# qingxu-thu/INSR-PDE

Hardware: AMD Instinct MI355X
Metric: collocation-points/sec/timestep (incl. ∇/Δ residual + Adam) at 1/2/4/8 GPUs (higher is better)
Workload: dtype fp32

## Files before the change

### include/insr_siren.h

```cpp
#ifndef INSR_SIREN_H
#define INSR_SIREN_H

#ifdef __cplusplus
extern "C" {
#endif

#define INSR_MODE_VALUE 0
#define INSR_MODE_GRAD  1
#define INSR_MODE_LAP   2
#define INSR_MODE_MASK  0xF
#define INSR_MODE_PREC_SHIFT 4
#define INSR_JET_PREC(p) (((p) + 1) << INSR_MODE_PREC_SHIFT)
#define INSR_MODE_BPREC_SHIFT 12
#define INSR_JET_BPREC(p) (((p) + 1) << INSR_MODE_BPREC_SHIFT)
#define INSR_MODE_WSPLIT (1 << 8)
#define INSR_MODE_WIDE128 (1 << 9)
#define INSR_MODE_POLICY_SHIFT 16
#define INSR_JET_POLICY(p) (((p) + 1) << INSR_MODE_POLICY_SHIFT)
#define INSR_MODE_F16_SHIFT 19
#define INSR_JET_BWD_F16(m) (((m) + 1) << INSR_MODE_F16_SHIFT)
#define INSR_MODE_TILES_SHIFT 23
#define INSR_TILES_CODE(t) ((t) == 4 ? 3 : ((t) == 2 ? 2 : ((t) == 1 ? 1 : 0)))
#define INSR_MINB_256 0
#define INSR_MINB_512 1
#define INSR_MINB_128 2
#define INSR_MINB_1024 3
#define INSR_JET_TILES(f, b, minb) \
  ((INSR_TILES_CODE(f) | (INSR_TILES_CODE(b) << 2) | ((minb) << 4)) << INSR_MODE_TILES_SHIFT)

#define INSR_EINVAL   (-1)
#define INSR_EWIDTH   (-2)
#define INSR_ENOCOMM  (-3)
#define INSR_ECAPTURE (-4)
#define INSR_ERANGE   (-5)
#define INSR_ECOMM_BASE 1000

int insr_version(void);

const char* insr_build_id(void);

long insr_siren_param_count(int d_in, int d_out, int num_hidden, int width);

long insr_siren_wsplit_offset(int d_in, int d_out, int num_hidden, int width);
long insr_siren_wsplit_floats(int num_hidden, int width);
int insr_siren_wsplit(float* params, int d_in, int d_out, int num_hidden, int width, void* stream);
int insr_siren_wsplit_status(const float* params, int d_in, int d_out, int num_hidden, int width, void* stream);

int insr_siren_supported(int d_in, int d_out, int num_hidden, int width, int mode);

long insr_jet_act_bytes(long n_points, int d_in, int num_hidden, int width, int mode);

long insr_jet_partial_bytes(long n_points, int d_in, int d_out, int num_hidden, int width, int mode);

int insr_siren_jet_fwd(const float* x, long n_points, int d_in, int d_out, int num_hidden,
                       int width, int mode, const float* params, float* y, float* dy, float* lap,
                       float* act, void* stream);

#define INSR_MAX_FWD_JOBS 6
typedef struct InsrJetJob {
  const float* x;
  const float* params;
  float* y;
  float* dy;
  float* lap;
  float* act;
  long n;
  int d_out;
} InsrJetJob;
#define INSR_MIX_ADVECT 3
int insr_siren_jet_fwd_mixed(const InsrJetJob* jobs, const int* modes, const float* scalars, int n_jobs, int d_in,
                             int d_out, int num_hidden, int width, int prec_mode, void* stream);
int insr_siren_jet_fwd_multi(const InsrJetJob* jobs, int n_jobs, int d_in, int d_out,
                             int num_hidden, int width, int mode, void* stream);

int insr_siren_jet_bwd(const float* x, long n_points, int d_in, int d_out, int num_hidden,
                       int width, int mode, const float* params, const float* act,
                       const float* gy, const float* gdy, const float* glap, float* partial,
                       void* stream);

// ... 228 lines not shown
```

### insr-pde_amd/base/_native.py

```python
import contextlib
import ctypes
import os
import threading

import torch

_HERE = os.path.dirname(os.path.abspath(__file__))
LIB_PATH = os.environ.get("INSR_HIP_LIB", os.path.join(os.path.dirname(_HERE), "lib", "libinsr_hip.so"))

MODE_VALUE, MODE_GRAD, MODE_LAP = 0, 1, 2
MODE_MASK, MODE_PREC_SHIFT = 0xF, 4
MODE_WSPLIT = 1 << 8
PREC_F32, PREC_BF16X6, PREC_BF16X3, PREC_BF16, PREC_F16X3 = 0, 1, 2, 3, 4
PRECISIONS = {"fp32": PREC_F32, "bf16x6": PREC_BF16X6, "bf16x3": PREC_BF16X3, "bf16": PREC_BF16,
              "f16x3": PREC_F16X3}


def jet_prec(p):
    return (int(p) + 1) << MODE_PREC_SHIFT


MODE_BPREC_SHIFT = 12


# ... 94 lines not shown
    "insr_siren_jet_fwd": (_I, [_P, _L, _I, _I, _I, _I, _I, _P, _P, _P, _P, _P, _P]),
    "insr_siren_jet_fwd_multi": (_I, [_P, _I, _I, _I, _I, _I, _I, _P]),
    "insr_siren_jet_bwd": (_I, [_P, _L, _I, _I, _I, _I, _I, _P, _P, _P, _P, _P, _P, _P]),
    "insr_jet_partial_blocks": (_I, [_L, _I, _I, _I]),
    "insr_siren_jet_bwd_grad": (_I, [_P, _L, _I, _I, _I, _I, _I, _P, _P, _P, _P, _P, _P, _P, _I, _P]),
    "insr_jet_bwd_work_bytes": (_L, [_L, _I, _I, _I, _I, _I]),
    "insr_siren_jet_bwd_grad_multi": (_I, [_P, _I, _I, _I, _I, _I, _I, _P, _P, _P, _I, _P]),
    "insr_jet_bwd_multi_work_bytes": (_L, [_P, _I, _I, _I, _I, _I, _I]),
    "insr_siren_jet_bwd_multi_rows": (_I, [_P, _I, _I, _I, _I, _I, _I, _P, _P, _P]),
    "insr_siren_jet_bwd_multi_sweep": (_I, [_P, _I, _I, _I, _I, _I, _I, _P, _P, _P]),
    "insr_jet_bwd_is_wide": (_I, [_L, _I, _I, _I]),
    "insr_jet_bwd_path": (_I, [_L, _I, _I, _I, _I, _I]),
    "insr_jet_bwd_kernel": (_I, [_L, _I, _I, _I, _I, _I]),
    "insr_comm_available": (_I, []),
    "insr_comm_id_bytes": (_L, []),
    "insr_comm_unique_id": (_I, [_P]),
    "insr_comm_init": (_I, [_P, _I, _I, _P]),
    "insr_comm_allreduce_sum": (_I, [_P, _P, _L, _P]),
    "insr_comm_destroy": (_I, [_P]),
    "insr_jet_split_tiles": (_I, [_L, _I, _I, _I, _I]),
    "insr_sq_loss_work_floats": (_L, []),
    "insr_svd_energy_work_floats": (_L, []),
    "insr_svd_energy_fwd": (_I, [_P, _L, _I, _F, _F, _P, _P, _P]),
    "insr_svd_energy_bwd": (_I, [_P, _L, _I, _F, _F, _P, _P, _P]),
    "insr_elastic_work_floats": (_L, []),
    "insr_elastic_energy": (_I, [_P, _P, _P]),
    "insr_sq_loss_fwd": (_I, [_I, _P, _P, _P, _P, _L, _I, _F, _F, _F, _F, _F, _P, _P, _P]),
    "insr_sq_loss_group": (_I, [_P, _I, _P, _P]),
    "insr_axpy_clamp": (_I, [_P, _P, _F, _F, _F, _P, _L, _P]),
    "insr_siren_wsplit_offset": (_L, [_I, _I, _I, _I]),
    "insr_siren_wsplit_floats": (_L, [_I, _I]),
    "insr_siren_wsplit": (_I, [_P, _I, _I, _I, _I, _P]),
    "insr_siren_wsplit_status": (_I, [_P, _I, _I, _I, _I, _P]),
    "insr_siren_jet_fwd_mixed": (_I, [_P, _P, _P, _I, _I, _I, _I, _I, _I, _P]),
    "insr_adam_step_nets": (_I, [_I, _P, _P, _P, _P, _P, _P, _P, _F, _F, _F, _I, _P]),
    "insr_adam_plateau_step_nets": (_I, [_I, _P, _P, _P, _P, _P, _P, _P, _F, _F, _F, _P, _I, _P]),
    "insr_adam_step_partials": (_I, [_P, _I, _L, _P, _I, _P, _P, _P, _L, _P, _P, _F, _F, _F, _P, _I, _P]),
    "insr_siren_jet_bwd_grad_adam": (_I, [_P, _L, _I, _I, _I, _I, _I, _P, _P, _P, _P, _P, _P, _P, _I, _I, _P, _P, _P,
                                          _F, _F, _F, _P, _I, _P]),
    "insr_jet_wide_launch_threads": (_I, [_L, _I, _I, _I, _I, _I, _P]),
    "insr_sq_loss_bwd": (_I, [_I, _P, _P, _P, _P, _L, _I, _F, _F, _F, _F, _F, _P, _P, _P, _P, _P, _P]),
    "insr_reduce_partials": (_I, [_P, _I, _L, _P, _I, _P]),
    "insr_reduce_partials_strided": (_I, [_P, _I, _L, _L, _P, _I, _P]),
    "insr_jet_partial_stride": (_L, [_I, _I, _I, _I]),
    "insr_adam_prepare": (_I, [_P, _F, _F, _P]),
    "insr_plateau_step": (_I, [_P, _P, _I, _I, _P]),
    "insr_adam_step_multi": (_I, [_I, _P, _P, _P, _P, _P, _P, _F, _F, _F, _I, _P]),
    "insr_sampler_state_bytes": (_L, []),
    "insr_sample_boxes": (_I, [_P, _I, _I, ctypes.c_ulonglong, _P, _P]),
    "insr_sample_boxes_rep": (_I, [_P, _I, _I, _I, _P, ctypes.c_ulonglong, _P, _P]),
    "insr_advect1d_rows": (_L, [_L]),
    "insr_advect1d_iteration": (_I, [_P, _P, _I, _I, _L, _L, _P, _P, _F, _F, _F, _F, ctypes.c_ulonglong, _P, _P,
                                     _P, _L, _P, _P, _P]),
    "insr_adam_step": (_I, [_P, _P, _P, _P, _L, _P, _F, _F, _F, _P]),
    "insr_jet_bwd_seed_rows": (_I, [_L, _I, _I, _I, _I, _I]),
    "insr_siren_jet_bwd_seeded": (_I, [_P, _L, _I, _I, _I, _I, _I, _P, _P, _P, _P, _P, _P, _I, _P, _P, _P]),
    "insr_reduce_partials_fin": (_I, [_P, _I, _L, _L, _P, _I, _P, _P]),
    "insr_adam_step_partials_fin": (_I, [_P, _I, _L, _P, _I, _P, _P, _P, _L, _P, _P, _F, _F, _F, _P, _I, _P, _P]),
    "insr_siren_jet_bwd_grad_adam_fin": (_I, [_P, _L, _I, _I, _I, _I, _I, _P, _P, _P, _I, _P, _P, _P, _F, _F, _F, _P,
                                              _I, _P, _P]),
}


MAX_FWD_JOBS = 6


# ... 127 lines not shown
```

### insr-pde_amd/csrc/capi.hip

```cpp
#include <cstdlib>
#include <map>
#include <mutex>
#include <tuple>

#include "jet_common.hpp"
#include "optim.hpp"

namespace insr {

int streams_for(int din, int mode) {
  if (mode == INSR_MODE_VALUE) return 1;
  if (mode == INSR_MODE_GRAD) return 1 + din;
  if (mode == INSR_MODE_LAP) return 2 + din;
  return -1;
}

int nt_for(int width) {
  if (width == 32) return 2;
  if (width == 64) return 4;
  if (width == 128) return 8;
  if (width == 256) return 16;
  return -1;
}

// ... 463 lines not shown
  bool resident(long n, int L) const { return use_resident(n, S, NT, lap, nqb, L, k); }
  bool recompute(int L) const { return use_fb(S, NT, lap, nqb, L, k); }
  bool resident_f16(long n, int L) const { return resident(n, L) && use_resident_f16(n, S, NT, lap, nqb, L, k); }
  int path(long n, int L) const { return recompute(L) ? 3 : (resident(n, L) ? 2 : (wide(n) ? 1 : 0)); }
};

}

using namespace insr;

extern "C" {

int insr_version(void) { return 300; }

long insr_siren_param_count(int din, int dout, int L, int W) {
  return (long)W * din + W + (long)L * ((long)W * W + W) + (long)dout * W + dout;
}

long insr_jet_partial_stride(int din, int dout, int L, int W) {
  return (insr_siren_param_count(din, dout, L, W) + 3) & ~3L;
}

long insr_siren_wsplit_offset(int din, int dout, int L, int W) {
  if (!shape_ok(din, dout, L, W, 0)) return INSR_EINVAL;
  return wsplit_offset(din, dout, L, W);
}
long insr_siren_wsplit_floats(int L, int W) {
  if (L < 0 || nt_for(W) < 0) return INSR_EINVAL;
  return wsplit_total_floats(L, W);
}
int insr_siren_wsplit(float* params, int din, int dout, int L, int W, void* stream) {
  if (!params || !shape_ok(din, dout, L, W, 0)) return INSR_EINVAL;
  return wsplit_launch(params, din, dout, L, W, params + wsplit_offset(din, dout, L, W), (hipStream_t)stream);
}

namespace {
struct Scratch {
  void* ptr = nullptr;
  size_t bytes = 0;
};
std::mutex g_scratch_mu;
std::map<std::tuple<int, hipStream_t, int>, Scratch> g_scratch;
}

static const float* with_planes(const float* params, int din, int dout, int L, int W, int mode, hipStream_t st,
                                int slot, int* rc) {
  *rc = 0;
  if ((mode & INSR_MODE_WSPLIT) || L < 1) return params;
  const long pc = insr_siren_param_count(din, dout, L, W);
  const size_t bytes = (size_t)(wsplit_offset(din, dout, L, W) + wsplit_total_floats(L, W)) * sizeof(float);
  int dev = 0;
  (void)hipGetDevice(&dev);
  std::lock_guard<std::mutex> lk(g_scratch_mu);
  Scratch& e = g_scratch[std::make_tuple(dev, st, slot)];
  if (e.bytes < bytes) {
    hipStreamCaptureStatus cs = hipStreamCaptureStatusNone;
    (void)hipStreamIsCapturing(st, &cs);
    if (cs != hipStreamCaptureStatusNone) {
      *rc = INSR_ECAPTURE;
      return nullptr;
    }
    if (e.ptr) (void)hipFree(e.ptr);
    e.ptr = nullptr;
    e.bytes = 0;
    if (hipMalloc(&e.ptr, bytes) != hipSuccess) {
      *rc = (int)hipErrorOutOfMemory;
// ... 892 lines not shown
```

### insr-pde_amd/csrc/jet_common.hpp

```cpp
#pragma once
#include <hip/hip_runtime.h>
#include <stdint.h>

#include "../../include/insr_siren.h"

typedef float floatx4 __attribute__((ext_vector_type(4)));

#define OMEGA 30.0f
#define OMEGA2 900.0f
#define OMEGA3 27000.0f

namespace insr {


__host__ __device__ inline long act_tiles(long n) { return ((n + 63) / 64) * 4; }

__device__ __forceinline__ floatx4 mfma4(float a, float b, floatx4 c) {
  return __builtin_amdgcn_mfma_f32_16x16x4f32(a, b, c, 0, 0, 0);
}

__host__ __device__ inline long hidden_off(int din, int W, int j) {
  return (long)W * din + W + (long)(j - 1) * ((long)W * W + W);
}
__host__ __device__ inline long out_off(int din, int W, int L) {
// ... 19 lines not shown
__host__ __device__ inline long wsplit_total_floats(int L, int W) { return 5L * L * W * W + 4; }

inline int device_cus() {
  static const int c = [] {
    int dev = 0, v = 0;
    (void)hipGetDevice(&dev);
    return (hipDeviceGetAttribute(&v, hipDeviceAttributeMultiprocessorCount, dev) != hipSuccess || v <= 0) ? 256 : v;
  }();
  return c;
}

__device__ __forceinline__ float* act_base(float* act, int layer, int ntiles, int tile, int S, int NT) {
  return act + ((long)layer * ntiles + tile) * (long)(S * NT) * 256;
}
__device__ __forceinline__ const float* act_base(const float* act, int layer, int ntiles, int tile, int S,
                                                 int NT) {
  return act + ((long)layer * ntiles + tile) * (long)(S * NT) * 256;
}

template <int CTRL>
__device__ __forceinline__ float add_dpp(float v) {
  const int o = __builtin_amdgcn_update_dpp(0, __builtin_bit_cast(int, v), CTRL, 0xF, 0xF, false);
  return v + __builtin_bit_cast(float, o);
}

__device__ __forceinline__ float sum16(float v) {
  v = add_dpp<0xB1>(v);
  v = add_dpp<0x4E>(v);
  v = add_dpp<0x141>(v);
  v = add_dpp<0x140>(v);
  return v;
}

constexpr float kFastArgMax = 8192.0f;

__device__ __forceinline__ float revs_reduced(float x) {
  const float n = rintf(x * 0.15915494309189535f);
  float r = fmaf(-n, 6.28125f, x);
  r = fmaf(-n, 1.9353071795864769e-3f, r);
  return r * 0.15915494309189535f;
}

__device__ __forceinline__ void sincos_fast(float x, float& s, float& c) {
  const float t = revs_reduced(x);
  s = __builtin_amdgcn_sinf(t);
  c = __builtin_amdgcn_cosf(t);
}

__device__ __forceinline__ float sin_fast(float x) { return __builtin_amdgcn_sinf(revs_reduced(x)); }

__device__ __forceinline__ bool wave_any_big(float amax) {
  return __any(amax > kFastArgMax);
}

template <int CTRL>
__device__ __forceinline__ float max_dpp(float v) {
  const int o = __builtin_amdgcn_update_dpp(0, __builtin_bit_cast(int, v), CTRL, 0xF, 0xF, false);
  return fmaxf(v, __builtin_bit_cast(float, o));
}
__device__ __forceinline__ float wave_max_nn(float v) {
  v = max_dpp<0xB1>(v);
  v = max_dpp<0x4E>(v);
  v = max_dpp<0x141>(v);
  v = max_dpp<0x140>(v);
  const int b = __builtin_bit_cast(int, v);
  const unsigned r0 = (unsigned)__builtin_amdgcn_readlane(b, 0), r1 = (unsigned)__builtin_amdgcn_readlane(b, 16);
  const unsigned r2 = (unsigned)__builtin_amdgcn_readlane(b, 32), r3 = (unsigned)__builtin_amdgcn_readlane(b, 48);
  const unsigned m01 = r0 > r1 ? r0 : r1, m23 = r2 > r3 ? r2 : r3;
  return __builtin_bit_cast(float, m01 > m23 ? m01 : m23);
}

__device__ __forceinline__ float wave_max(float v) {
#pragma unroll
  for (int o = 32; o >= 1; o >>= 1) v = fmaxf(v, __shfl_xor(v, o, 64));
  return v;
}


template <int NT, int S, bool LAP, bool FAST>
__device__ __forceinline__ void sine_jet_impl(floatx4 (&a)[NT][S]) {
  constexpr int NTAN = LAP ? S - 2 : S - 1;
#pragma unroll
  for (int rt = 0; rt < NT; ++rt) {
#pragma unroll
    for (int r = 0; r < 4; ++r) {
      const float arg = OMEGA * a[rt][0][r];
      float sn, cs;
      if constexpr (S == 1) {
        if constexpr (FAST) sn = sin_fast(arg); else sn = sinf(arg);
        a[rt][0][r] = sn;
        continue;
      }
      if constexpr (FAST) sincos_fast(arg, sn, cs); else sincosf(arg, &sn, &cs);
      const float wc = OMEGA * cs;
      if constexpr (LAP) {
        float t2 = 0.f;
#pragma unroll
        for (int i = 0; i < NTAN; ++i) t2 = fmaf(a[rt][1 + i][r], a[rt][1 + i][r], t2);
        a[rt][S - 1][r] = wc * a[rt][S - 1][r] - OMEGA2 * sn * t2;
      }
#pragma unroll
      for (int i = 0; i < NTAN; ++i) a[rt][1 + i][r] *= wc;
// ... 336 lines not shown
  const float* gdy[kBwdJobs];
  const float* glap[kBwdJobs];
  int n[kBwdJobs];
  int nbal[kBwdJobs];
  int first[kBwdJobs + 1];
  int njobs;
  SeedTab seeds;
};
template <int NQ>
int dispatch_bwd_q(int NT, int S, bool LAP, int T, const BwdJobsX6* jobs, int din, int dout, int L,
                   const float* prm, float* part, long P, hipStream_t st);
struct AdamArgs {
  float* p = nullptr;
  float* m = nullptr;
  float* v = nullptr;
  float* st = nullptr;
  const float* loss = nullptr;
  int patience = 0;
  float b1 = 0.f, b2 = 0.f, eps = 0.f;
  int shape[4] = {0, 0, 0, 0};
  LossFin fin;
};

struct FbJobs;
template <int NQ>
int dispatch_wide_bwd_q(int NT, int S, bool LAP, const FbJobs& J, int N, int din, int dout, int L, const float* prm,
                        float* work, float* grad, int accumulate, int f16, int phases, const AdamArgs& A,
                        hipStream_t st);
long wide_work_floats(long n, int din, int dout, int L, int W, int S);
template <int NQ>
int dispatch_fwd_mixed_q(int NT, int din, const InsrJetJob* jobs, const int* modes, const float* scalars, int njobs,
                         int dout, int L, hipStream_t st);
int wsplit_launch(const float* prm, int din, int dout, int L, int W, float* planes, hipStream_t st);
void wide_launch_threads(long n, int din, int dout, int L, int W, int S, long* out);
int dispatch_resident_bwd(int S, bool LAP, int L, const float* x, int N, int din, int dout, const float* prm,
                          const float* act, const float* gy, const float* gdy, const float* glap, float* work,
                          float* grad, int accumulate, hipStream_t st);
long resident_work_floats(long n, int din, int dout, int L);
int resident_blocks(long n);

struct FbJobs {
  const float* x[kBwdJobs];
  const float* act[kBwdJobs];
  const float* gy[kBwdJobs];
  const float* gdy[kBwdJobs];
  const float* glap[kBwdJobs];
  int n[kBwdJobs];
  int tstart[kBwdJobs + 1];
  int njobs;
  SeedTab seeds;
};
constexpr int kFbSeedTiles = 24;
int dispatch_fb_bwd(int S, bool LAP, int L, const FbJobs& J, int din, int dout, const float* prm, float* work,
                    float* grad, int accumulate, int saved, int phases, const AdamArgs& A, hipStream_t st);
bool fb_supported(int S, bool LAP, int L);
bool fb_saved_supported(int S, bool LAP, int L);
long fb_work_floats(long tiles, int din, int dout, int L);
int fb_launch_blocks(long tiles);

#define INSR_DISPATCH(NTV, FN, ...)                \
  switch (S * 2 + (LAP ? 1 : 0)) {                 \
    case 2: return FN<NTV, 1, false>(__VA_ARGS__); \
    case 4: return FN<NTV, 2, false>(__VA_ARGS__); \
    case 6: return FN<NTV, 3, false>(__VA_ARGS__); \
    case 8: return FN<NTV, 4, false>(__VA_ARGS__); \
    case 7: return FN<NTV, 3, true>(__VA_ARGS__);  \
// ... 7 lines not shown
```

### insr-pde_amd/csrc/jet_fb.hpp

```cpp
#pragma once
#include <type_traits>

#include "jet_x6w.hpp"

namespace insr {

constexpr int kFbSmallMax = 1412;

#ifdef INSR_STAMPS
constexpr int kFbStampPts = 32;
static __device__ unsigned long long g_fb_stamps[8 * 8 * kFbStampPts];
#define FB_STAMP(k)                                                                                     \
  do {                                                                                                 \
    if (blockIdx.x == 0 && lane == 0 && tile - t0 < 8)                                                 \
      g_fb_stamps[((wave * 8 + (tile - t0)) * kFbStampPts) + (k)] = __builtin_amdgcn_s_memtime();     \
  } while (0)
#else
#define FB_STAMP(k) \
  do {              \
  } while (0)
#endif

template <int S, int L, int ZR, bool SAVED = false, bool SEED = false>
struct FbGeo {
  using BG = X6BwdGeo<4, 8>;
  static constexpr int NZL = (!SAVED && (L - ZR) > 0) ? (L - ZR) : 0;
  static constexpr size_t P_BYTES = (size_t)S * BG::ZSET * 2;
  static constexpr size_t H_BYTES = (size_t)S * BG::ZSET * 2;
  static constexpr size_t ZS_BYTES = (size_t)NZL * S * 8 * 64 * 16;
  static constexpr int SW_FLOATS = 128 * 3 + 128 + L * 128 + 3 * 128;
  static constexpr size_t SW_OFF = P_BYTES + H_BYTES + ZS_BYTES;
  static constexpr size_t SACC_OFF = SW_OFF + (size_t)SW_FLOATS * 4;
  static constexpr size_t SEED_OFF = SACC_OFF + (size_t)kFbSmallMax * 4;
  static constexpr size_t MX_OFF = SEED_OFF + (size_t)S * 3 * 16 * 4;
  static constexpr size_t SSEED_OFF = MX_OFF + 2 * 5 * 8 * 4;
  static constexpr size_t BYTES = SSEED_OFF + (SEED ? ((size_t)kFbSeedTiles * S * 48 + 8 * INSR_SEED_MAX) * 4 : 0);
};

struct FbSinCos {
  floatx4 s, c;
};
__device__ __noinline__ FbSinCos fb_sincos_libm(floatx4 z) {
  FbSinCos o;
#pragma unroll
  for (int r = 0; r < 4; ++r) {
    float a, b;
    sincosf(OMEGA * z[r], &a, &b);
    o.s[r] = a;
    o.c[r] = b;
  }
  return o;
}
__device__ __forceinline__ void fb_sincos(const floatx4& z, floatx4& s, floatx4& c) {
  float amax = 0.f;
#pragma unroll
  for (int r = 0; r < 4; ++r) amax = fmaxf(amax, fabsf(OMEGA * z[r]));
  if (wave_any_big(amax)) {
    const FbSinCos o = fb_sincos_libm(z);
    s = o.s;
    c = o.c;
    return;
  }
#pragma unroll
  for (int r = 0; r < 4; ++r) {
    float a, b;
    sincos_fast(OMEGA * z[r], a, b);
// ... 148 lines not shown
      for (int w = 0; w < 8; ++w)
#pragma unroll
        for (int q = 0; q < INSR_SEED_MAX; ++q) r[q] += swq[w * INSR_SEED_MAX + q];
      *reinterpret_cast<floatx4*>(J.seeds.lpart + (long)blockIdx.x * INSR_SEED_MAX) = r;
    }
  }

  __syncthreads();

  for (int tile = t0; tile < t1; ++tile) {
    int zo = 0, po = 0, tid = threadIdx.x;
    asm volatile("" : "+s"(zo), "+s"(po));
    asm volatile("" : "+v"(tid));
    const float* prmt = prm + po;
    const int wave = __builtin_amdgcn_readfirstlane(tid >> 6), lane = tid & 63, g = lane >> 4, c = lane & 15;
    const int rt = wave;
    const int ra = wave >> 1, cb = wave & 1;
    const int n0 = 16 * rt + 4 * g;
    const u32x4* wsp = wsp_base(prmt, din, dout, L, W);
    unsigned char* lbt = lb + zo;
    unsigned short* P = reinterpret_cast<unsigned short*>(lbt);
    unsigned short* H = reinterpret_cast<unsigned short*>(lbt + GG::P_BYTES);
    floatx4* ZS = reinterpret_cast<floatx4*>(lbt + GG::P_BYTES + GG::H_BYTES);
    const float* sw = reinterpret_cast<const float*>(lbt + GG::SW_OFF);
    const float* W0s = sw;
    const float* b0s = sw + 3 * W;
    const float* bhs = sw + 4 * W;
    const float* Wos = sw + (4 + L) * W;
    float* sacc = reinterpret_cast<float*>(lbt + GG::SACC_OFF);
    float* seed = reinterpret_cast<float*>(lbt + GG::SEED_OFF);
    float* mx = reinterpret_cast<float*>(lbt + GG::MX_OFF);
    auto exchange = [&](float (&m)[5], auto ncls) __attribute__((always_inline)) {
      constexpr int NC = decltype(ncls)::value;
#pragma unroll
      for (int k = 0; k < NC; ++k) m[k] = wave_max_nn(m[k]);
      if (lane < NC) {
        float v = m[0];
#pragma unroll
        for (int k = 1; k < NC; ++k) v = lane == k ? m[k] : v;
        mx[(slot * 5 + lane) * 8 + wave] = v;
      }
      __syncthreads();
#pragma unroll
      for (int k = 0; k < NC; ++k) {
        const floatx4 a = *reinterpret_cast<const floatx4*>(mx + (slot * 5 + k) * 8);
        const floatx4 b = *reinterpret_cast<const floatx4*>(mx + (slot * 5 + k) * 8 + 4);
        const float v = fmaxf(fmaxf(fmaxf(a[0], a[1]), fmaxf(a[2], a[3])), fmaxf(fmaxf(b[0], b[1]), fmaxf(b[2], b[3])));
        m[k] = __builtin_bit_cast(float, __builtin_amdgcn_readfirstlane(__builtin_bit_cast(int, v)));
      }
      slot ^= 1;
    };

    int k = 0;
#pragma unroll
    for (int q = 1; q < kBwdJobs; ++q) k += (q < J.njobs && tile >= J.tstart[q]) ? 1 : 0;
    const int lt = tile - J.tstart[k];
    const int N = J.n[k];
    const int p = lt * 16 + c;
    const bool valid = p < N;
    const float* __restrict__ x = J.x[k];
    float xk[3];
#pragma unroll
    for (int kk = 0; kk < 3; ++kk) xk[kk] = (valid && kk < din) ? x[(long)p * din + kk] : 0.f;
    FB_STAMP(0);
    float sdv = 0.f;
    float gsd[(SAVED && !SEED) ? S : 1][3];
    if constexpr (SAVED && !SEED) {
#pragma unroll
      for (int s = 0; s < S; ++s)
#pragma unroll
        for (int o = 0; o < 3; ++o) {
          float v = 0.f;
          if (valid && o < dout) {
            const float* g0 = s == 0 ? J.gy[k] : ((LAP && s == S - 1) ? J.glap[k] : J.gdy[k]);
            const long at = (s == 0 || (LAP && s == S - 1)) ? (long)p * dout + o : ((long)p * dout + o) * din + (s - 1);
            if (g0) v = g0[at];
          }
          gsd[s][o] = v;
        }
    }
    const float* actk = SAVED ? J.act[k] : nullptr;
// ... 72 lines not shown
#pragma unroll
      for (int kc = 0; kc < KC; ++kc) {
        const FragQ<4> wc = wf;
        if (kc + 1 < KC) wf = wsp_frag<4, NT>(wsl, L, 0, j, rt, kc + 1, lane);
#pragma unroll
        for (int s = 0; s < S; ++s) {
          const FragQ<4> bf = lds_frag<4, ZPLANE>(P + s * ZSET + c * LDB + 32 * kc + 8 * g);
          acc[s] = mfma_q<4>(wc, bf, acc[s]);
          X6_SCHED_FENCE();
        }
      }
#pragma unroll
      for (int s = 0; s < S; ++s) a[s] = acc[s] * (s == 0 ? usv : ((LAP && s == S - 1) ? usl : ust));
      FB_STAMP(2 * j);
      if constexpr (j <= NZL) {
#pragma unroll
        for (int s = 0; s < S; ++s) ZS[(((j - 1) * S + s) * 8 + wave) * 64 + lane] = a[s];
      } else {
#pragma unroll
        for (int s = 0; s < S; ++s) zr[j - NZL - 1][s] = a[s];
      }
      if constexpr (j < L) {
        wpre = wsp_frag<4, NT>(wsl, L, 0, j + 1, rt, 0, lane);
        put_h(jc, j == L - 1);
      }
      FB_STAMP(2 * j + 1);
    };
    if constexpr (L >= 1) fwd_layer(std::integral_constant<int, 1>{});
    if constexpr (L >= 2) fwd_layer(std::integral_constant<int, 2>{});
    if constexpr (L >= 3) fwd_layer(std::integral_constant<int, 3>{});
    if constexpr (L >= 4) fwd_layer(std::integral_constant<int, 4>{});
    }

    floatx4 zc[S];
    if constexpr (SAVED) {
      zload(L, zc);
    } else {
#pragma unroll
      for (int s = 0; s < S; ++s) zc[s] = zr[ZR - 1][s];
    }
    floatx4 sn, cs;
    fb_sincos(zc[0], sn, cs);
    floatx4 hb[S];
#pragma unroll
    for (int s = 0; s < S; ++s) hb[s] = floatx4{0.f, 0.f, 0.f, 0.f};
    for (int o = 0; o < dout; ++o) {
      float ga[S];
#pragma unroll
      for (int s = 0; s < S; ++s) {
        if constexpr (!SAVED)
          ga[s] = seed[(s * 3 + o) * 16 + c];
        else if constexpr (SEED)
          ga[s] = reinterpret_cast<const float*>(lbt + GG::SSEED_OFF)[(((tile - t0) * S + s) * 3 + o) * 16 + c];
        else
          ga[s] = o == 0 ? gsd[s][0] : (o == 1 ? gsd[s][1] : gsd[s][2]);
      }
      const floatx4 w4 = *reinterpret_cast<const floatx4*>(Wos + (o * W + n0));
      floatx4 acc4 = floatx4{0.f, 0.f, 0.f, 0.f};
#pragma unroll
      for (int s = 0; s < S; ++s) {
        const floatx4 hs = fb_h<S, LAP>(s, zc, sn, cs);
#pragma unroll
        for (int r = 0; r < 4; ++r) {
          acc4[r] = fmaf(ga[s], hs[r], acc4[r]);
          hb[s][r] = fmaf(w4[r], ga[s], hb[s][r]);
        }
      }
#pragma unroll
      for (int r = 0; r < 4; ++r) {
        const float v = sum16(acc4[r]);
        if (c == 0) sacc[so + (long)o * W + n0 + r] += v;
      }
      if (wave == 0) {
        const float v = sum16(g == 0 ? ga[0] : 0.f);
        if (lane == 0) sacc[so + (long)dout * W + o] += v;
      }
    }

    FB_STAMP(10);
    auto bwd_layer = [&](auto jc) __attribute__((always_inline)) {
      constexpr int j = decltype(jc)::value;
      constexpr int sp = 11 + 5 * (L - j);
      const u32x4* wsl = wsp;
      floatx4 zp[S];
      if constexpr (SAVED && j > 1) zload(j - 1, zp);
      sine_rev<S, LAP>(hb, zc, sn, cs);
#pragma unroll
      for (int r = 0; r < 4; ++r) {
        const float v = sum16(hb[0][r]);
        if (c == 0) sacc[sb + (long)(j - 1) * W + n0 + r] += v;
      }
      if constexpr (j == 1) {
#pragma unroll
        for (int r = 0; r < 4; ++r) {
          const int n = n0 + r;
          float z = b0s[n];
    #pragma unroll
      for (int kk = 0; kk < 3; ++kk)
        if (kk < din) z = fmaf(W0s[3 * n + kk], xk[kk], z);
          zp[0][r] = z;
#pragma unroll
          for (int i = 0; i < NTAN; ++i) zp[1 + i][r] = W0s[3 * n + i];
          if constexpr (LAP) zp[S - 1][r] = 0.f;
        }
      } else if constexpr (SAVED) {
      } else if constexpr (j - 1 <= NZL) {
#pragma unroll
        for (int s = 0; s < S; ++s) zp[s] = ZS[(((j - 2) * S + s) * 8 + wave) * 64 + lane];
      } else {
#pragma unroll
        for (int s = 0; s < S; ++s) zp[s] = zr[j - 1 - NZL - 1][s];
      }
      float m[5] = {0.f, 0.f, 0.f, 0.f, 0.f};
#pragma unroll
      for (int s = 0; s < S; ++s)
#pragma unroll
        for (int r = 0; r < 4; ++r) {
          const int cl = s == 0 ? 0 : ((LAP && s == S - 1) ? 2 : 1);
          m[cl] = fmaxf(m[cl], fabsf(hb[s][r]));
        }
      if constexpr (SAVED && S > 1) fb_h_bounds<S, LAP>(zp, m[3], m[4]);
      FB_STAMP(sp);
      exchange(m, std::integral_constant<int, (S == 1 ? 1 : (SAVED ? 5 : (LAP ? 3 : 2)))>{});
      FB_STAMP(sp + 1);
      int eht = 0, ehl = 0;
      if constexpr (SAVED) {
        if constexpr (S > 1) eht = f16_exp_for(m[3]);
        if constexpr (LAP) ehl = f16_exp_for(m[4]);
      } else {
        if constexpr (S > 1) eht = eh[j - 1][0];
        if constexpr (LAP) ehl = eh[j - 1][1];
      }
      const float bht = ldexpf(1.f, eht), bhl = ldexpf(1.f, ehl);
      const float zht = ldexpf(1.f, -eht), zhl = ldexpf(1.f, -ehl);
      int e = f16_exp_for(fmaxf(m[0], fmaxf(m[1] * zht, m[2] * zhl)));
      if (E[j - 1] != kNoE) {
        e = min(e, E[j - 1] + 60);
        if (e != E[j - 1]) {
          const float f = ldexpf(1.f, e - E[j - 1]);
#pragma unroll
          for (int ct = 0; ct < NT; ++ct) dacc[j - 1][ct] *= f;
        }
      }
      E[j - 1] = e;
      const float zsc = ldexpf(1.f, e);
      const int col = c * LDB + n0;
      {
        floatx4 snp, csp;
        fb_sincos(zp[0], snp, csp);
#pragma unroll
        for (int s = 0; s < S; ++s) {
        const float f2 = s == 0 ? 1.f : ((LAP && s == S - 1) ? zhl : zht);
        const floatx4 v = (hb[s] * zsc) * f2;
        lds_put4<4, ZPLANE>(P + s * ZSET + col, v[0], v[1], v[2], v[3]);
          floatx4 h = fb_h<S, LAP>(s, zp, snp, csp);
        if (s > 0) h *= (LAP && s == S - 1) ? bhl : bht;
        lds_put4<4, ZPLANE>(H + s * ZSET + col, h[0], h[1], h[2], h[3]);
        }
      }
      __syncthreads();
      FB_STAMP(sp + 2);
      FragQ<4> wn = wsp_frag<4, NT>(wsl, L, 1, j, rt, 0, lane);
#pragma unroll
      for (int ch = 0; ch < NCH; ++ch) {
        const int u = 2 * ch + (g >> 1);
        const bool live = u < S;
        const int p0 = 8 * (g & 1);
        FragQ<4> af[2];
#pragma unroll
        for (int i = 0; i < 2; ++i) {
          const unsigned short* pa =
              P + (live ? u : 0) * ZSET + (p0 + (c >> 2)) * LDB + 16 * (2 * ra + i) + 4 * (c & 3);
#pragma unroll
          for (int q = 0; q < 2; ++q) {
            const v4s lo = ds_read_tr16(pa + q * ZPLANE);
            const v4s hi = ds_read_tr16(pa + q * ZPLANE + 4 * LDB);
            const u32x2 wl = __builtin_bit_cast(u32x2, lo), wh = __builtin_bit_cast(u32x2, hi);
            af[i].q[q] = live ? u32x4{wl[0], wl[1], wh[0], wh[1]} : u32x4{0u, 0u, 0u, 0u};
          }
        }
        auto bfrag = [&](int q4) __attribute__((always_inline)) {
// ... 18 lines not shown
          for (int i = 0; i < 2; ++i) dacc[j - 1][4 * i + q4] = mfma_q<4>(af[i], bf, dacc[j - 1][4 * i + q4]);
          X6_SCHED_FENCE();
          if (q4 < 3) bf = bn;
        }
      }
      FB_STAMP(sp + 3);
      if (tile == t1 - 1) {
        floatx4* out = reinterpret_cast<floatx4*>(dpart + ((long)(j - 1) * nb + blockIdx.x) * W * W);
        const float f = ldexpf(1.f, -E[j - 1]);
#pragma unroll
        for (int q = 0; q < NT; ++q) out[((2 * ra + q / 4) * NT + 4 * cb + q % 4) * 64 + lane] = dacc[j - 1][q] * f;
      }
      floatx4 nh[S];
#pragma unroll
      for (int s = 0; s < S; ++s) nh[s] = floatx4{0.f, 0.f, 0.f, 0.f};
      FragQ<4> pb = lds_frag<4, ZPLANE>(P + c * LDB + 8 * g);
#pragma unroll
      for (int kc = 0; kc < KC; ++kc) {
        const FragQ<4> wt = wn;
        if (kc + 1 < KC) wn = wsp_frag<4, NT>(wsl, L, 1, j, rt, kc + 1, lane);
#pragma unroll
        for (int s = 0; s < S; ++s) {
          const int nk = s + 1 < S ? kc : kc + 1, ns = s + 1 < S ? s + 1 : 0;
          FragQ<4> pn;
          if (nk < KC) pn = lds_frag<4, ZPLANE>(P + ns * ZSET + c * LDB + 32 * nk + 8 * g);
          nh[s] = mfma_q<4>(wt, pb, nh[s]);
          X6_SCHED_FENCE();
          if (nk < KC) pb = pn;
        }
      }
      const float zun = ldexpf(1.f, -e) / kF16WScale;
#pragma unroll
      for (int s = 0; s < S; ++s) hb[s] = (nh[s] * zun) * (s == 0 ? 1.f : ((LAP && s == S - 1) ? bhl : bht));
#pragma unroll
      for (int s = 0; s < S; ++s) zc[s] = zp[s];
      fb_sincos(zc[0], sn, cs);
      FB_STAMP(sp + 4);
    };
    if constexpr (L >= 5) bwd_layer(std::integral_constant<int, 5>{});
    if constexpr (L >= 4) bwd_layer(std::integral_constant<int, 4>{});
    if constexpr (L >= 3) bwd_layer(std::integral_constant<int, 3>{});
    if constexpr (L >= 2) bwd_layer(std::integral_constant<int, 2>{});
    bwd_layer(std::integral_constant<int, 1>{});

    sine_rev<S, LAP>(hb, zc, sn, cs);
#pragma unroll
    for (int r = 0; r < 4; ++r) {
      const float v = sum16(hb[0][r]);
      if (c == 0) sacc[(long)W * din + n0 + r] += v;
    }
#pragma unroll
    for (int kk = 0; kk < 3; ++kk) {
      if (kk >= din) break;
#pragma unroll
      for (int r = 0; r < 4; ++r) {
        float v = hb[0][r] * xk[kk];
#pragma unroll
        for (int i = 0; i < NTAN; ++i)
          if (i == kk) v += hb[1 + i][r];
        v = sum16(v);
        if (c == 0) sacc[(long)(n0 + r) * din + kk] += v;
      }
    }
    FB_STAMP(31);
  }

  if (t1 == t0) {
    const int wave = threadIdx.x >> 6, lane = threadIdx.x & 63, ra = wave >> 1, cb = wave & 1;
#pragma unroll
    for (int jl = 0; jl < L; ++jl) {
      floatx4* out = reinterpret_cast<floatx4*>(dpart + ((long)jl * nb + blockIdx.x) * W * W);
#pragma unroll
      for (int q = 0; q < NT; ++q) out[((2 * ra + q / 4) * NT + 4 * cb + q % 4) * 64 + lane] = dacc[jl][q];
    }
  }
  __syncthreads();
  for (int i = threadIdx.x; i < Ps; i += 512) small[(long)blockIdx.x * Ps + i] = sacc0[i];
}

inline int fb_blocks(long tiles) {
  const long cus = device_cus();
  if (tiles <= cus) return (int)(tiles > 0 ? tiles : 1);
  const long per = (tiles + cus - 1) / cus;
  return (int)((tiles + per - 1) / per);
}

inline long fb_work_floats_impl(long tiles, int din, int dout, int L) {
  const long nb = fb_blocks(tiles);
  return (long)L * nb * 128 * 128 + nb * small_count(din, dout, L, 128);
}

template <int S, bool LAP, int L, int ZR, bool SAVED>
int fb_bwd_t(const FbJobs& J, int din, int dout, const float* prm, float* work, float* grad, int accumulate,
             int phases, const AdamArgs& A, hipStream_t st) {
// ... 46 lines not shown
```

### insr-pde_amd/csrc/jet_x6.hpp

```cpp
#pragma once
#include "jet_split.hpp"

namespace insr {

typedef short bf16x8 __attribute__((ext_vector_type(8)));
typedef unsigned u32x4 __attribute__((ext_vector_type(4)));
typedef unsigned u32x2 __attribute__((ext_vector_type(2)));
typedef __bf16 bf16x2v __attribute__((ext_vector_type(2)));

__device__ __forceinline__ unsigned pk_bf16(float a, float b) {
  const bf16x2v v = {(__bf16)a, (__bf16)b};
  return __builtin_bit_cast(unsigned, v);
}
__device__ __forceinline__ float bf_lo(unsigned p) { return __builtin_bit_cast(float, p << 16); }
__device__ __forceinline__ float bf_hi(unsigned p) { return __builtin_bit_cast(float, p & 0xffff0000u); }

__device__ __forceinline__ void split3(float a, float b, unsigned& h, unsigned& m, unsigned& l) {
  h = pk_bf16(a, b);
  float ra = a - bf_lo(h), rb = b - bf_hi(h);
  m = pk_bf16(ra, rb);
  ra -= bf_lo(m);
  rb -= bf_hi(m);
  l = pk_bf16(ra, rb);
}

template <int NQ>
constexpr int np_of() { return NQ == 4 ? 2 : NQ; }

template <int NQ>
struct FragQ {
  u32x4 q[np_of<NQ>()];
};

typedef _Float16 f16x2v __attribute__((ext_vector_type(2)));
typedef _Float16 f16x8 __attribute__((ext_vector_type(8)));
__device__ __forceinline__ unsigned pk_f16(float a, float b) {
  const f16x2v v = {(_Float16)a, (_Float16)b};
  return __builtin_bit_cast(unsigned, v);
}
using Frag3 = FragQ<3>;

template <int NQ>
__device__ __forceinline__ void splitq(float a, float b, unsigned (&o)[np_of<NQ>()]) {
  if constexpr (NQ == 4) {
    o[0] = pk_f16(a, b);
    const f16x2v h = __builtin_bit_cast(f16x2v, o[0]);
    o[1] = pk_f16(a - (float)h[0], b - (float)h[1]);
    return;
  }
  o[0] = pk_bf16(a, b);
  if constexpr (NQ > 1) {
    float ra = a - bf_lo(o[0]), rb = b - bf_hi(o[0]);
    o[1] = pk_bf16(ra, rb);
    if constexpr (NQ > 2) {
      ra -= bf_lo(o[1]);
      rb -= bf_hi(o[1]);
      o[2] = pk_bf16(ra, rb);
    }
  }
}

template <int NQ>
__device__ __forceinline__ FragQ<NQ> split_frag(const floatx4& v0, const floatx4& v1) {
  unsigned t[4][np_of<NQ>()];
  splitq<NQ>(v0[0], v0[1], t[0]);
  splitq<NQ>(v0[2], v0[3], t[1]);
  splitq<NQ>(v1[0], v1[1], t[2]);
  splitq<NQ>(v1[2], v1[3], t[3]);
  FragQ<NQ> f;
#pragma unroll
  for (int q = 0; q < np_of<NQ>(); ++q) f.q[q] = u32x4{t[0][q], t[1][q], t[2][q], t[3][q]};
  return f;
}

__device__ __forceinline__ floatx4 mfma_bf(const u32x4& a, const u32x4& b, floatx4 c) {
  return __builtin_amdgcn_mfma_f32_16x16x32_bf16(__builtin_bit_cast(bf16x8, a), __builtin_bit_cast(bf16x8, b), c,
                                                 0, 0, 0);
}

__device__ __forceinline__ floatx4 mfma_h(const u32x4& a, const u32x4& b, floatx4 c) {
// ... 1161 lines not shown
```

### insr-pde_amd/csrc/jet_x6w.hip

```cpp
#include "jet_x6w.hpp"

namespace insr {
template int dispatch_wide_bwd_q<3>(int, int, bool, const FbJobs&, int, int, int, int, const float*, float*, float*, int, int, int,
                                    const AdamArgs&, hipStream_t);
long wide_work_floats(long n, int din, int dout, int L, int W, int S) {
  return wide_work_floats_impl(n, din, dout, L, W, S);
}
int wsplit_launch(const float* prm, int din, int dout, int L, int W, float* planes, hipStream_t st) {
  if (L < 1) return 0;
  const long threads = 4L * L * (W / 16) * (W / 32) * 64;
  const dim3 grid((unsigned)((threads + 255) / 256));
  u32x4* out = reinterpret_cast<u32x4*>(planes);
  unsigned* status = reinterpret_cast<unsigned*>(planes + 5L * L * W * W);
  if (const int rc = (int)hipMemsetAsync(status, 0, 4 * sizeof(unsigned), st)) return rc;
  switch (W) {
    case 32: hipLaunchKernelGGL((wsplit_kernel<2>), grid, dim3(256), 0, st, prm, din, L, out, status); break;
    case 64: hipLaunchKernelGGL((wsplit_kernel<4>), grid, dim3(256), 0, st, prm, din, L, out, status); break;
    case 128: hipLaunchKernelGGL((wsplit_kernel<8>), grid, dim3(256), 0, st, prm, din, L, out, status); break;
    case 256: hipLaunchKernelGGL((wsplit_kernel<16>), grid, dim3(256), 0, st, prm, din, L, out, status); break;
    default: return INSR_EWIDTH;
  }
  (void)dout;
  return (int)hipGetLastError();
}
void wide_launch_threads(long n, int din, int dout, int L, int W, int S, long* out) {
  wide_launch_threads_impl(n, din, dout, L, W, S, out);
}
}
```

Measured before the change: 111.3 million.

## Tighten fused backward reductions, double-buffer sine state, and use mixed-FMA f16 split

Several micro-optimisations land in the fused backward kernel. Per-class wave max reductions are merged into one interleaved DPP/permlane pass on unsigned bit patterns, and four-row sum16 calls become a single vectorised sum16x4 with b128 shared-memory accumulates. Pre-activations and sin/cos are double-buffered across layers so the per-layer copy and recomputation of sincos goes away. The f16 residual split now uses v_fma_mix_f32 inline asm, and a standalone probe kernel exposes that split for testing. Risks include the unsigned max being valid only for non-negative floats and extra register pressure from the double buffers.

After: 115.9 million, median of 6. 1.04x the previous value.

```diff
diff --git a/include/insr_siren.h b/include/insr_siren.h
--- a/include/insr_siren.h
+++ b/include/insr_siren.h
@@ -45,6 +45,7 @@
 long insr_siren_wsplit_floats(int num_hidden, int width);
 int insr_siren_wsplit(float* params, int d_in, int d_out, int num_hidden, int width, void* stream);
 int insr_siren_wsplit_status(const float* params, int d_in, int d_out, int num_hidden, int width, void* stream);
+int insr_split_f16(const float* in, unsigned* hi, unsigned* lo, long n_pairs, void* stream);
 
 int insr_siren_supported(int d_in, int d_out, int num_hidden, int width, int mode);
 
diff --git a/insr-pde_amd/base/_native.py b/insr-pde_amd/base/_native.py
--- a/insr-pde_amd/base/_native.py
+++ b/insr-pde_amd/base/_native.py
@@ -150,6 +150,7 @@
     "insr_siren_wsplit_floats": (_L, [_I, _I]),
     "insr_siren_wsplit": (_I, [_P, _I, _I, _I, _I, _P]),
     "insr_siren_wsplit_status": (_I, [_P, _I, _I, _I, _I, _P]),
+    "insr_split_f16": (_I, [_P, _P, _P, _L, _P]),
     "insr_siren_jet_fwd_mixed": (_I, [_P, _P, _P, _I, _I, _I, _I, _I, _I, _P]),
     "insr_adam_step_nets": (_I, [_I, _P, _P, _P, _P, _P, _P, _P, _F, _F, _F, _I, _P]),
     "insr_adam_plateau_step_nets": (_I, [_I, _P, _P, _P, _P, _P, _P, _P, _F, _F, _F, _P, _I, _P]),
diff --git a/insr-pde_amd/csrc/capi.hip b/insr-pde_amd/csrc/capi.hip
--- a/insr-pde_amd/csrc/capi.hip
+++ b/insr-pde_amd/csrc/capi.hip
@@ -519,6 +519,11 @@
 int insr_siren_wsplit(float* params, int din, int dout, int L, int W, void* stream) {
   if (!params || !shape_ok(din, dout, L, W, 0)) return INSR_EINVAL;
   return wsplit_launch(params, din, dout, L, W, params + wsplit_offset(din, dout, L, W), (hipStream_t)stream);
+}
+
+int insr_split_f16(const float* in, unsigned* hi, unsigned* lo, long npairs, void* stream) {
+  if (npairs < 0 || npairs > (1L << 31) || (npairs && (!in || !hi || !lo))) return INSR_EINVAL;
+  return split_f16_probe_launch(in, hi, lo, npairs, (hipStream_t)stream);
 }
 
 namespace {
diff --git a/insr-pde_amd/csrc/jet_common.hpp b/insr-pde_amd/csrc/jet_common.hpp
--- a/insr-pde_amd/csrc/jet_common.hpp
+++ b/insr-pde_amd/csrc/jet_common.hpp
@@ -75,6 +75,18 @@
   return v;
 }
 
+__device__ __forceinline__ floatx4 sum16x4(floatx4 v) {
+#pragma unroll
+  for (int r = 0; r < 4; ++r) v[r] = add_dpp<0xB1>(v[r]);
+#pragma unroll
+  for (int r = 0; r < 4; ++r) v[r] = add_dpp<0x4E>(v[r]);
+#pragma unroll
+  for (int r = 0; r < 4; ++r) v[r] = add_dpp<0x141>(v[r]);
+#pragma unroll
+  for (int r = 0; r < 4; ++r) v[r] = add_dpp<0x140>(v[r]);
+  return v;
+}
+
 constexpr float kFastArgMax = 8192.0f;
 
 __device__ __forceinline__ float revs_reduced(float x) {
@@ -97,20 +109,44 @@
 }
 
 template <int CTRL>
-__device__ __forceinline__ float max_dpp(float v) {
-  const int o = __builtin_amdgcn_update_dpp(0, __builtin_bit_cast(int, v), CTRL, 0xF, 0xF, false);
-  return fmaxf(v, __builtin_bit_cast(float, o));
-}
-__device__ __forceinline__ float wave_max_nn(float v) {
-  v = max_dpp<0xB1>(v);
-  v = max_dpp<0x4E>(v);
-  v = max_dpp<0x141>(v);
-  v = max_dpp<0x140>(v);
-  const int b = __builtin_bit_cast(int, v);
-  const unsigned r0 = (unsigned)__builtin_amdgcn_readlane(b, 0), r1 = (unsigned)__builtin_amdgcn_readlane(b, 16);
-  const unsigned r2 = (unsigned)__builtin_amdgcn_readlane(b, 32), r3 = (unsigned)__builtin_amdgcn_readlane(b, 48);
-  const unsigned m01 = r0 > r1 ? r0 : r1, m23 = r2 > r3 ? r2 : r3;
-  return __builtin_bit_cast(float, m01 > m23 ? m01 : m23);
+__device__ __forceinline__ unsigned umax_dpp(unsigned keep, unsigned give) {
+  const unsigned o = (unsigned)__builtin_amdgcn_update_dpp(0, (int)give, CTRL, 0xF, 0xF, true);
+  return keep > o ? keep : o;
+}
+__device__ __forceinline__ unsigned umax_rows(unsigned v) {
+  const auto r = __builtin_amdgcn_permlane16_swap(v, v, false, false);
+  v = r[0] > r[1] ? r[0] : r[1];
+  const auto q = __builtin_amdgcn_permlane32_swap(v, v, false, false);
+  return q[0] > q[1] ? q[0] : q[1];
+}
+template <int NC>
+__device__ __forceinline__ unsigned wave_umax_classes(const unsigned (&u)[5], int lane) {
+  unsigned r;
+  if constexpr (NC > 1) {
+    const bool b0 = lane & 1, b1 = lane & 2;
+    const unsigned r01 = umax_dpp<0xB1>(b0 ? u[1] : u[0], b0 ? u[0] : u[1]);
+    if constexpr (NC > 2) {
+      const unsigned r23 = umax_dpp<0xB1>(b0 ? u[3] : u[2], b0 ? u[2] : u[3]);
+      r = umax_dpp<0x4E>(b1 ? r23 : r01, b1 ? r01 : r23);
+    } else {
+      r = umax_dpp<0x4E>(r01, r01);
+    }
+  } else {
+    r = umax_dpp<0xB1>(u[0], u[0]);
+    r = umax_dpp<0x4E>(r, r);
+  }
+  r = umax_dpp<0x124>(r, r);
+  r = umax_dpp<0x128>(r, r);
+  r = umax_rows(r);
+  if constexpr (NC > 4) {
+    unsigned q = umax_dpp<0xB1>(u[4], u[4]);
+    q = umax_dpp<0x4E>(q, q);
+    q = umax_dpp<0x124>(q, q);
+    q = umax_dpp<0x128>(q, q);
+    q = umax_rows(q);
+    r = lane == 4 ? q : r;
+  }
+  return r;
 }
 
 __device__ __forceinline__ float wave_max(float v) {
@@ -513,6 +549,7 @@
 int dispatch_fwd_mixed_q(int NT, int din, const InsrJetJob* jobs, const int* modes, const float* scalars, int njobs,
                          int dout, int L, hipStream_t st);
 int wsplit_launch(const float* prm, int din, int dout, int L, int W, float* planes, hipStream_t st);
+int split_f16_probe_launch(const float* in, unsigned* hi, unsigned* lo, long npairs, hipStream_t st);
 void wide_launch_threads(long n, int din, int dout, int L, int W, int S, long* out);
 int dispatch_resident_bwd(int S, bool LAP, int L, const float* x, int N, int din, int dout, const float* prm,
                           const float* act, const float* gy, const float* gdy, const float* glap, float* work,
diff --git a/insr-pde_amd/csrc/jet_fb.hpp b/insr-pde_amd/csrc/jet_fb.hpp
--- a/insr-pde_amd/csrc/jet_fb.hpp
+++ b/insr-pde_amd/csrc/jet_fb.hpp
@@ -32,6 +32,7 @@
   static constexpr size_t SW_OFF = P_BYTES + H_BYTES + ZS_BYTES;
   static constexpr size_t SACC_OFF = SW_OFF + (size_t)SW_FLOATS * 4;
   static constexpr size_t SEED_OFF = SACC_OFF + (size_t)kFbSmallMax * 4;
+  static_assert(SACC_OFF % 16 == 0, "the compact row's b128 updates (bias and output-layer sums)");
   static constexpr size_t MX_OFF = SEED_OFF + (size_t)S * 3 * 16 * 4;
   static constexpr size_t SSEED_OFF = MX_OFF + 2 * 5 * 8 * 4;
   static constexpr size_t BYTES = SSEED_OFF + (SEED ? ((size_t)kFbSeedTiles * S * 48 + 8 * INSR_SEED_MAX) * 4 : 0);
@@ -246,21 +247,19 @@
     float* mx = reinterpret_cast<float*>(lbt + GG::MX_OFF);
     auto exchange = [&](float (&m)[5], auto ncls) __attribute__((always_inline)) {
       constexpr int NC = decltype(ncls)::value;
-#pragma unroll
-      for (int k = 0; k < NC; ++k) m[k] = wave_max_nn(m[k]);
-      if (lane < NC) {
-        float v = m[0];
-#pragma unroll
-        for (int k = 1; k < NC; ++k) v = lane == k ? m[k] : v;
-        mx[(slot * 5 + lane) * 8 + wave] = v;
-      }
+      unsigned* mxu = reinterpret_cast<unsigned*>(mx);
+      unsigned u[5];
+#pragma unroll
+      for (int k = 0; k < 5; ++k) u[k] = k < NC ? __builtin_bit_cast(unsigned, m[k]) : 0u;
+      const unsigned w = wave_umax_classes<NC>(u, lane);
+      if (lane < NC) mxu[(slot * 5 + lane) * 8 + wave] = w;
       __syncthreads();
 #pragma unroll
       for (int k = 0; k < NC; ++k) {
-        const floatx4 a = *reinterpret_cast<const floatx4*>(mx + (slot * 5 + k) * 8);
-        const floatx4 b = *reinterpret_cast<const floatx4*>(mx + (slot * 5 + k) * 8 + 4);
-        const float v = fmaxf(fmaxf(fmaxf(a[0], a[1]), fmaxf(a[2], a[3])), fmaxf(fmaxf(b[0], b[1]), fmaxf(b[2], b[3])));
-        m[k] = __builtin_bit_cast(float, __builtin_amdgcn_readfirstlane(__builtin_bit_cast(int, v)));
+        const u32x4 a = *reinterpret_cast<const u32x4*>(mxu + (slot * 5 + k) * 8);
+        const u32x4 b = *reinterpret_cast<const u32x4*>(mxu + (slot * 5 + k) * 8 + 4);
+        const unsigned v = max(max(max(a[0], a[1]), max(a[2], a[3])), max(max(b[0], b[1]), max(b[2], b[3])));
+        m[k] = __builtin_bit_cast(float, __builtin_amdgcn_readfirstlane((int)v));
       }
       slot ^= 1;
     };
@@ -399,15 +398,17 @@
     if constexpr (L >= 4) fwd_layer(std::integral_constant<int, 4>{});
     }
 
-    floatx4 zc[S];
-    if constexpr (SAVED) {
-      zload(L, zc);
-    } else {
-#pragma unroll
-      for (int s = 0; s < S; ++s) zc[s] = zr[ZR - 1][s];
-    }
-    floatx4 sn, cs;
-    fb_sincos(zc[0], sn, cs);
+    floatx4 zq[2][S], snq[2], csq[2];
+    {
+      floatx4(&zc)[S] = zq[0];
+      if constexpr (SAVED) {
+        zload(L, zc);
+      } else {
+#pragma unroll
+        for (int s = 0; s < S; ++s) zc[s] = zr[ZR - 1][s];
+      }
+      fb_sincos(zc[0], snq[0], csq[0]);
+    }
     floatx4 hb[S];
 #pragma unroll
     for (int s = 0; s < S; ++s) hb[s] = floatx4{0.f, 0.f, 0.f, 0.f};
@@ -426,18 +427,15 @@
       floatx4 acc4 = floatx4{0.f, 0.f, 0.f, 0.f};
 #pragma unroll
       for (int s = 0; s < S; ++s) {
-        const floatx4 hs = fb_h<S, LAP>(s, zc, sn, cs);
+        const floatx4 hs = fb_h<S, LAP>(s, zq[0], snq[0], csq[0]);
 #pragma unroll
         for (int r = 0; r < 4; ++r) {
           acc4[r] = fmaf(ga[s], hs[r], acc4[r]);
           hb[s][r] = fmaf(w4[r], ga[s], hb[s][r]);
         }
       }
-#pragma unroll
-      for (int r = 0; r < 4; ++r) {
-        const float v = sum16(acc4[r]);
-        if (c == 0) sacc[so + (long)o * W + n0 + r] += v;
-      }
+      acc4 = sum16x4(acc4);
+      if (c == 0) *reinterpret_cast<floatx4*>(sacc + so + (long)o * W + n0) += acc4;
       if (wave == 0) {
         const float v = sum16(g == 0 ? ga[0] : 0.f);
         if (lane == 0) sacc[so + (long)dout * W + o] += v;
@@ -449,13 +447,16 @@
       constexpr int j = decltype(jc)::value;
       constexpr int sp = 11 + 5 * (L - j);
       const u32x4* wsl = wsp;
-      floatx4 zp[S];
+      constexpr int qc = (L - j) & 1;
+      floatx4(&zc)[S] = zq[qc];
+      floatx4(&zp)[S] = zq[qc ^ 1];
+      const floatx4 &sn = snq[qc], &cs = csq[qc];
+      floatx4 &snp = snq[qc ^ 1], &csp = csq[qc ^ 1];
       if constexpr (SAVED && j > 1) zload(j - 1, zp);
       sine_rev<S, LAP>(hb, zc, sn, cs);
-#pragma unroll
-      for (int r = 0; r < 4; ++r) {
-        const float v = sum16(hb[0][r]);
-        if (c == 0) sacc[sb + (long)(j - 1) * W + n0 + r] += v;
+      {
+        const floatx4 v = sum16x4(hb[0]);
+        if (c == 0) *reinterpret_cast<floatx4*>(sacc + sb + (long)(j - 1) * W + n0) += v;
       }
       if constexpr (j == 1) {
 #pragma unroll
@@ -513,7 +514,6 @@
       const float zsc = ldexpf(1.f, e);
       const int col = c * LDB + n0;
       {
-        floatx4 snp, csp;
         fb_sincos(zp[0], snp, csp);
 #pragma unroll
         for (int s = 0; s < S; ++s) {
@@ -598,9 +598,6 @@
       const float zun = ldexpf(1.f, -e) / kF16WScale;
 #pragma unroll
       for (int s = 0; s < S; ++s) hb[s] = (nh[s] * zun) * (s == 0 ? 1.f : ((LAP && s == S - 1) ? bhl : bht));
-#pragma unroll
-      for (int s = 0; s < S; ++s) zc[s] = zp[s];
-      fb_sincos(zc[0], sn, cs);
       FB_STAMP(sp + 4);
     };
     if constexpr (L >= 5) bwd_layer(std::integral_constant<int, 5>{});
@@ -609,23 +606,26 @@
     if constexpr (L >= 2) bwd_layer(std::integral_constant<int, 2>{});
     bwd_layer(std::integral_constant<int, 1>{});
 
-    sine_rev<S, LAP>(hb, zc, sn, cs);
-#pragma unroll
-    for (int r = 0; r < 4; ++r) {
-      const float v = sum16(hb[0][r]);
-      if (c == 0) sacc[(long)W * din + n0 + r] += v;
+    sine_rev<S, LAP>(hb, zq[L & 1], snq[L & 1], csq[L & 1]);
+    {
+      const floatx4 v = sum16x4(hb[0]);
+      if (c == 0) *reinterpret_cast<floatx4*>(sacc + (long)W * din + n0) += v;
     }
 #pragma unroll
     for (int kk = 0; kk < 3; ++kk) {
       if (kk >= din) break;
+      floatx4 v;
 #pragma unroll
       for (int r = 0; r < 4; ++r) {
-        float v = hb[0][r] * xk[kk];
+        v[r] = hb[0][r] * xk[kk];
 #pragma unroll
         for (int i = 0; i < NTAN; ++i)
-          if (i == kk) v += hb[1 + i][r];
-        v = sum16(v);
-        if (c == 0) sacc[(long)(n0 + r) * din + kk] += v;
+          if (i == kk) v[r] += hb[1 + i][r];
+      }
+      v = sum16x4(v);
+      if (c == 0) {
+#pragma unroll
+        for (int r = 0; r < 4; ++r) sacc[(long)(n0 + r) * din + kk] += v[r];
       }
     }
     FB_STAMP(31);
diff --git a/insr-pde_amd/csrc/jet_x6.hpp b/insr-pde_amd/csrc/jet_x6.hpp
--- a/insr-pde_amd/csrc/jet_x6.hpp
+++ b/insr-pde_amd/csrc/jet_x6.hpp
@@ -44,8 +44,10 @@
 __device__ __forceinline__ void splitq(float a, float b, unsigned (&o)[np_of<NQ>()]) {
   if constexpr (NQ == 4) {
     o[0] = pk_f16(a, b);
-    const f16x2v h = __builtin_bit_cast(f16x2v, o[0]);
-    o[1] = pk_f16(a - (float)h[0], b - (float)h[1]);
+    float ra, rb;
+    asm("v_fma_mix_f32 %0, %1, -1.0, %2 op_sel_hi:[1,0,0]" : "=v"(ra) : "v"(o[0]), "v"(a));
+    asm("v_fma_mix_f32 %0, %1, -1.0, %2 op_sel:[1,0,0] op_sel_hi:[1,0,0]" : "=v"(rb) : "v"(o[0]), "v"(b));
+    o[1] = pk_f16(ra, rb);
     return;
   }
   o[0] = pk_bf16(a, b);
diff --git a/insr-pde_amd/csrc/jet_x6w.hip b/insr-pde_amd/csrc/jet_x6w.hip
--- a/insr-pde_amd/csrc/jet_x6w.hip
+++ b/insr-pde_amd/csrc/jet_x6w.hip
@@ -23,6 +23,22 @@
   (void)dout;
   return (int)hipGetLastError();
 }
+static __global__ __launch_bounds__(256) void split_f16_probe_kernel(const float* __restrict__ in,
+                                                                     unsigned* __restrict__ hi,
+                                                                     unsigned* __restrict__ lo, long npairs) {
+  const long i = (long)blockIdx.x * 256 + threadIdx.x;
+  if (i >= npairs) return;
+  unsigned t[2];
+  splitq<4>(in[2 * i], in[2 * i + 1], t);
+  hi[i] = t[0];
+  lo[i] = t[1];
+}
+int split_f16_probe_launch(const float* in, unsigned* hi, unsigned* lo, long npairs, hipStream_t st) {
+  if (npairs <= 0) return 0;
+  hipLaunchKernelGGL(split_f16_probe_kernel, dim3((unsigned)((npairs + 255) / 256)), dim3(256), 0, st, in, hi, lo,
+                     npairs);
+  return (int)hipGetLastError();
+}
 void wide_launch_threads(long n, int din, int dout, int L, int W, int S, long* out) {
   wide_launch_threads_impl(n, din, dout, L, W, S, out);
 }
```
